# zhuhaozh/metadrive_ped

Hardware: AMD Instinct MI355X
Metric: agent-steps/sec at 4096 envs x 240-beam lidar (higher is better)
Workload: dtype f32; 1 GPU; BASELINE configs[1]: 4096 batched MetaDriveEnv per GPU, 3-block PG map (reference default block distribution: curves, straights, ramps, X/T intersections, roundabouts), 240-beam lidar, traffic_density=0.1, trigger traffic, auto-reset; envs_per_gpu=4096, agents_per_env=1, mover_capacity=24, n_beams=240

## Files before the change

### include/md_entity.h

```cpp
#ifndef MD_ENTITY_H
#define MD_ENTITY_H

#include <stddef.h>

#include "md_geom.h"
#include "md_lane_change.h"

MD_HD int md_scene_of_env(const MdState* g, int e) { return g->scene_of ? g->scene_of[e] : e; }
MD_HD size_t md_track_stride(const MdState* s, const MdConfig* c) {
    return (size_t)(s->walk.n_scenes > 0 ? s->walk.n_scenes : c->n_envs) * (size_t)c->cap;
}
MD_HD int md_scene(const MdState* s, int e) { return s->scene_of ? s->scene_of[0] : e; }

MD_HD MdState md_env_view(const MdState* g, const MdConfig* c, int e) {
    MdState v = *g;
    const size_t b = (size_t)e * (size_t)c->cap;
    const size_t bs = (size_t)md_scene_of_env(g, e) * (size_t)c->cap;
    const size_t a = (size_t)e * (size_t)c->agents_per_env;
    v.shape = g->shape + b;
    v.dyn = g->dyn ? g->dyn + b : 0;
    v.param = g->param ? g->param + b : 0;
    v.nav = g->nav ? g->nav + b : 0;
    v.pid = g->pid ? g->pid + b : 0;
    v.action = g->action ? g->action + 2 * b : 0;
// ... 118 lines not shown
    s->action[2 * n] = steer;
    s->action[2 * n + 1] = thr;
    float yaw = (sh->s * d->last_c - sh->c * d->last_s) / (float)c->substeps;
    d->last_x = sh->cx;
    d->last_y = sh->cy;
    d->last_c = sh->c;
    d->last_s = sh->s;
    d->steering = steer;
    d->throttle = thr;
    float x = sh->cx, y = sh->cy, psi = d->heading, v = d->speed;
    MdBicycle bike;
    md_bicycle_prepare(steer, thr, v, sh->hl, sh->hw, c->dt, c->enable_reverse && (sh->flags & MD_F_AGENT), &s->param[n], &bike);
    float c0, s0;
    md_sincos(psi, &s0, &c0);
    float cp = c0 * bike.cb - s0 * bike.sb, sp = s0 * bike.cb + c0 * bike.sb;
    for (int k = 0; k < c->substeps; ++k) md_bicycle_substep(&x, &y, &psi, &v, &cp, &sp, &yaw, thr, &bike, &s->param[n], c->dt);
    sh->cx = x;
    sh->cy = y;
    d->heading = psi;
    d->speed = v;
    md_sincos(psi, &sh->s, &sh->c);
}


#define MD_OBS_TASKS 9

typedef struct MdObsCtx {
    const MdLane *lane, *ref0, *ref_last, *next0, *fin, *rl;
    float cur_w, cur_n, positive_road;
    int valid;
    int cur_block;
} MdObsCtx;

MD_HD void md_observe_ctx(const MdLane* lanes, const MdRoad* roads, const MdState* s, int n, MdObsCtx* k) {
    const MdShape* sh = &s->shape[n];
    const MdNav* nav = &s->nav[n];
    k->valid = md_drives(sh->flags) && nav->lane >= 0;
    k->lane = k->ref0 = k->ref_last = k->next0 = k->fin = k->rl = lanes;
    k->cur_w = k->cur_n = k->positive_road = 0.0f;
    k->cur_block = 0;
    if (!k->valid) return;
    const MdRoad* cur_road = &roads[nav->road0];
    k->cur_block = cur_road->block_kind;
    int has_next = nav->ck1 != nav->ck0;
    const MdRoad* next_road = has_next ? &roads[nav->road1] : cur_road;
    k->lane = &lanes[nav->lane];
    k->ref0 = &lanes[cur_road->first_lane];
    k->ref_last = &lanes[cur_road->first_lane + cur_road->n_lanes - 1];
    k->next0 = &lanes[next_road->first_lane];
    k->fin = &lanes[s->final_lane[n]];
    k->cur_w = k->lane->width;
    k->cur_n = (float)cur_road->n_lanes;
    k->positive_road = 1.0f;
    if (k->lane->road == nav->road0) k->rl = k->lane;
    else {
        k->rl = k->ref0;
        k->positive_road = cur_road->negative ? -1.0f : 1.0f;
    }
}

MD_HD void md_observe_task(int task, const MdObsCtx* k, const MdState* s, const MdConfig* c, int n, float* out5) {
    const MdShape* sh = &s->shape[n];
    const MdDyn* d = &s->dyn[n];
    float x = sh->cx, y = sh->cy;
    out5[0] = out5[1] = out5[2] = out5[3] = out5[4] = 0.0f;
    if (!k->valid) return;
    if (task == 0 || task == 2 || task == 5 || task == 6 || task == 7) {
        const MdLane* L = (task == 0) ? k->ref0 : ((task == 2) ? k->lane : ((task == 5) ? k->fin : k->rl));
        float px = (task == 6) ? d->last_x : x;
        float py = (task == 6) ? d->last_y : y;
        md_lane_local(L, px, py, &out5[0], &out5[1]);
    } else if (task == 3 || task == 4) {
        md_navi_for_checkpoint((task == 3) ? k->ref0 : k->next0, (k->cur_n / 2.0f - 0.5f) * k->cur_w, x, y, sh->c, sh->s,
                               k->cur_n, k->cur_w, c->curve_radius_max, c->curve_angle_max, out5);
    } else if (task == 1) {
        out5[0] = md_heading_diff(k->ref_last, x, y, sh->c, sh->s);
    } else if (task == 8) {
        float cosb = (sh->c * d->last_c + sh->s * d->last_s) / (md_norm(sh->c, sh->s) * md_norm(d->last_c, d->last_s));
        float beta = md_acos(md_clip(cosb, 0.0f, 1.0f));
        out5[0] = md_clip(beta / 0.1f, 0.0f, 1.0f);
        out5[1] = md_step_energy(md_fabs(d->speed) * 3.6f, md_norm(d->last_x - x, d->last_y - y));
    }
}

#define MD_OBS_LANES 16
#if defined(__HIP_DEVICE_COMPILE__)
#define MD_LANE_IN(lane, mask) __extension__({ unsigned long long m_; __asm__ volatile("s_mov_b64 %0, %1" : "=s"(m_) : "i"(mask)); __builtin_amdgcn_inverse_ballot_w64(m_); })
#else
#define MD_LANE_IN(lane, mask) ((((mask) >> (lane)) & 1ull) != 0)
#endif
#define MD_LANE_F(m) ((int)(offsetof(MdLane, m) / sizeof(float)))

// ... 123 lines not shown
    if (MD_LANE_IN(lane, MD_LY)) {
        num3 = ac_hi ? 2.0f * md_asin_small(n3) : MD_HALF_PI_F - md_asin_small(cosb);
        den3 = 0.1f;
    }
    if (MD_LANE_IN(lane, MD_LE)) {
        float t = 3.25f * md_exp(0.01f * (md_fabs(speed) * 3.6f));
        num3 = t * q1;
        den3 = 100.0f;
    }
    const float q3 = num3 / den3;

    int w0 = task * 5;
    MD_PICK2(MD_LN, out0, (q3 + 1.0f) / 2.0f, w0, w0 + (lane >= 10));
    MD_PICK(MD_LH, out0, (!(ln * n2 != 0.0f)) ? 0.0f : md_clip(q3, -1.0f, 1.0f) / 2.0f + 0.5f);
    MD_PICK(MD_LY, out0, q3);
    MD_PICK2(MD_LE, out0, q3 * 1000.0f, w0, w0 + 1);
    MD_PICK(MD_LB, w0, w0 + 2);
    MD_PICK(MD_LA, w0, w0 + 4);

    MD_PICK(0xFD18ull, out0, md_clip(out0, 0.0f, 1.0f));
    if (MD_LANE_IN(lane, 0xFFFFull)) r45[w0] = out0;
    if (MD_LANE_IN(lane, MD_LF | MD_LB)) r45[w0 + 1] = (lane >= 12) ? md_clip(out1, 0.0f, 1.0f) : out1;
#undef MD_PICK
#undef MD_PICK2
#undef MD_LF
#undef MD_LN
#undef MD_LH
#undef MD_LY
#undef MD_LE
#undef MD_LB
#undef MD_LA
}

MD_HD void md_route_borders(const MdObsCtx* k, const float (*r)[5], float* to_left, float* to_right) {
    *to_left = r[0][1] + k->cur_w / 2.0f;
    *to_right = k->cur_w * k->cur_n - *to_left;
}

MD_HD void md_observe_state_dims(const MdObsCtx* k, const MdState* s, const MdConfig* c, int n, const float (*r)[5], float* obs) {
    const MdDyn* d = &s->dyn[n];
    const int o_mid = md_obs_mid(c), o_ll = md_obs_ll(c), o_navi = md_obs_navi(c);
    float to_left, to_right;
    md_route_borders(k, r, &to_left, &to_right);
    float speed_kmh = md_fabs(d->speed) * 3.6f;
    const MdParam* P = &s->param[n];
    const int o_base = md_obs_base(c);
    if (o_base) {
        obs[0] = md_clip(2.0f * s->shape[n].hl / 10.0f, 0.0f, 1.0f);
        obs[1] = md_clip(2.0f * s->shape[n].hw / 2.5f, 0.0f, 1.0f);
    }
    if (c->n_side <= 0) {
        obs[o_base + 0] = md_clip(to_left / c->total_width, 0.0f, 1.0f);
        obs[o_base + 1] = md_clip(to_right / c->total_width, 0.0f, 1.0f);
    }
    obs[o_mid + 0] = r[1][0];
    obs[o_mid + 1] = md_clip((speed_kmh + 1.0f) / (P->max_speed_kmh + 1.0f), 0.0f, 1.0f);
    obs[o_mid + 2] = md_clip((d->steering / 60.0f + 1.0f) / 2.0f, 0.0f, 1.0f);
    obs[o_mid + 3] = md_clip((s->action[2 * n] + 1.0f) / 2.0f, 0.0f, 1.0f);
    obs[o_mid + 4] = md_clip((s->action[2 * n + 1] + 1.0f) / 2.0f, 0.0f, 1.0f);
    obs[o_mid + 5] = r[8][0];
    float llat = r[2][1];
    if (c->n_lane_line <= 0) obs[o_ll] = md_clip((llat * 2.0f / c->max_lane_width + 1.0f) / 2.0f, 0.0f, 1.0f);
    if (!md_is_tollgate(c))
        for (int i = 0; i < 5; ++i) {
            obs[o_navi + i] = r[3][i];
            obs[o_navi + 5 + i] = r[4][i];
        }
}

MD_HD void md_observe_combine(const MdObsCtx* k, const MdState* s, const MdConfig* c, int a, int env_just_reset,
                              const float (*r)[5]) {
    int n = a;
    int just_reset = env_just_reset || ((s->shape[n].flags & MD_F_SPAWNED) != 0);
    s->shape[n].flags &= ~MD_F_SPAWNED;
    int ai = a;
    float* obs = s->obs + (size_t)ai * c->obs_dim;
    float* info = s->step_info + (size_t)ai * 8;
    MdDyn* d = &s->dyn[n];
    MdNav* nav = &s->nav[n];
    const int toll = md_is_tollgate(c);
    if (!k->valid) {
        if (s->done_out) ((uint32_t*)s->done_out)[ai] = 0u;
        for (int i = 0; i < md_obs_lidar(c); ++i) obs[i] = 0.0f;
        for (int i = c->obs_dim - md_obs_tail(c); i < c->obs_dim; ++i) obs[i] = 0.0f;
        s->reward[ai] = 0.0f;
        s->cost[ai] = 0.0f;
        for (int i = 0; i < 8; ++i) info[i] = 0.0f;
        return;
    }
    float cur_w = k->cur_w, cur_n = k->cur_n;

    float to_left, to_right;
    md_route_borders(k, r, &to_left, &to_right);
    uint32_t fl = s->flags[n] & (MD_FL_CRASH_VEHICLE | MD_FL_CRASH_OBJECT | MD_FL_CRASH_HUMAN | MD_FL_CRASH_BUILDING |
                                 MD_FL_CRASH_SIDEWALK | MD_FL_ON_WHITE_CONT | MD_FL_ON_YELLOW_CONT | MD_FL_ON_BROKEN |
                                 MD_FL_ON_CROSSWALK | MD_FL_ON_LANE);
    if (to_right < 0.0f || to_left < 0.0f) fl |= MD_FL_OUT_OF_ROUTE;

    md_observe_state_dims(k, s, c, n, r, obs);
    float speed_kmh = md_fabs(d->speed) * 3.6f;
    const MdParam* P = &s->param[n];
    float ls = r[2][0], llat = r[2][1];

    float fs = r[5][0], flat = r[5][1];
    int arrive = (k->fin->length - 5.0f < fs) && (fs < k->fin->length + 5.0f) && (cur_w / 2.0f >= flat) &&
                 (flat >= (0.5f - cur_n) * cur_w);
    int out_of_road = !(fl & MD_FL_ON_LANE);
    if (c->out_of_route_done) out_of_road = out_of_road || (fl & MD_FL_OUT_OF_ROUTE);
    else if (c->on_continuous_line_done)
        out_of_road = out_of_road || (fl & (MD_FL_ON_YELLOW_CONT | MD_FL_ON_WHITE_CONT | MD_FL_CRASH_SIDEWALK));
    if (toll) {
        out_of_road = (fl & MD_FL_CRASH_SIDEWALK) != 0;
        if (c->on_continuous_line_done) out_of_road = out_of_road || (fl & MD_FL_ON_YELLOW_CONT);
    }
    if (c->is_multi_agent && c->ma_kind == MD_MA_PARKING_LOT)
        out_of_road = !(fl & MD_FL_ON_LANE) || (fl & (MD_FL_ON_YELLOW_CONT | MD_FL_CRASH_SIDEWALK));
    const int racing = c->is_multi_agent && c->ma_kind == MD_MA_RACING;
    if (racing)
        out_of_road = ls < -5.0f;
    if (arrive) fl |= MD_FL_ARRIVE_DEST;
    if (out_of_road) fl |= MD_FL_OUT_OF_ROAD;

    float positive_road = k->positive_road;
    float long_last = r[6][0], long_now = r[7][0], lateral_now = r[7][1];
    float lateral_factor = 1.0f;
    if (c->use_lateral_reward) lateral_factor = md_clip(1.0f - 2.0f * md_fabs(lateral_now) / cur_w, 0.0f, 1.0f);
    float reward = 0.0f;
    if (toll) {
        reward += c->driving_reward * (long_now - long_last) * lateral_factor;
        if (k->cur_block == '$') {
            if (k->lane->speed_limit < speed_kmh) reward = -c->overspeed_penalty * speed_kmh / P->max_speed_kmh;
        } else reward += c->speed_reward * (speed_kmh / P->max_speed_kmh);
    } else {
        reward += c->driving_reward * (long_now - long_last) * lateral_factor * positive_road;
        reward += c->speed_reward * (speed_kmh / P->max_speed_kmh) * positive_road;
    }
    float step_reward = reward;
    int idle = 0;
    if (racing && !just_reset && s->idle_ring) {
        float* ring = s->idle_ring + (size_t)ai * MD_IDLE_WINDOW;
        int cnt = nav->toll_state;
        ring[cnt % MD_IDLE_WINDOW] = md_fabs(long_now - long_last);
        cnt += 1;
        if (cnt >= 2 * MD_IDLE_WINDOW) cnt -= MD_IDLE_WINDOW;
        nav->toll_state = cnt;
        if (cnt >= MD_IDLE_WINDOW) {
            float sum = 0.0f;
            for (int i = 0; i < MD_IDLE_WINDOW; ++i) sum += ring[(cnt + i) % MD_IDLE_WINDOW];
            idle = sum < 0.1f;
        }
    }
    if (arrive) reward = c->success_reward;
    else if (out_of_road) reward = -c->out_of_road_penalty;
    else if (fl & MD_FL_CRASH_VEHICLE) reward = -c->crash_vehicle_penalty;
    else if (racing) {
        if (fl & MD_FL_CRASH_SIDEWALK) reward = -c->crash_sidewalk_penalty;
        else if (idle) reward = -c->idle_penalty;
    } else if (fl & MD_FL_CRASH_OBJECT) reward = -c->crash_object_penalty;

    float cost = 0.0f;
    if (out_of_road) cost = c->out_of_road_cost;
    else if (fl & MD_FL_CRASH_VEHICLE) cost = c->crash_vehicle_cost;
    else if (fl & MD_FL_CRASH_OBJECT) cost = c->crash_object_cost;

// ... 37 lines not shown
        if (max_step) fl |= MD_FL_TRUNCATED;
    }
    s->flags[n] = fl;
    s->reward[ai] = reward;
    s->cost[ai] = cost;
    if (s->done_out) ((uint32_t*)s->done_out)[ai] = md_done_word(fl);
    if (toll) {
        int t = nav->toll_state & 0xffffff, last = (nav->toll_state >> 24) & 0xff;
        const int cur = k->cur_block, in_toll = (cur == '$');
        if (in_toll) t += 1;
        obs[c->obs_dim - 2] = in_toll ? 1.0f : 0.0f;
        obs[c->obs_dim - 1] = (in_toll && t > c->min_pass_steps) ? 1.0f : 0.0f;
        if (last && last != cur) {
            if (in_toll) nav->toll_entry = nav->steps + 1;
            else if ((cur == 'y' || cur == 'Y') && last == '$') nav->toll_exit = nav->steps + 1;
        }
        last = cur;
        nav->toll_state = t | (last << 24);
    }

    float step_energy = just_reset ? 0.0f : r[8][1];
    s->pid[n].energy += step_energy;
    info[0] = step_reward;
    info[1] = md_fabs(d->speed);
    info[2] = step_energy;
    info[3] = s->pid[n].energy;
    info[4] = just_reset ? 0.0f : info[4] + reward;
    info[5] = just_reset ? 0.0f : info[5] + cost;
    (void)llat;
    info[6] = ls;
    info[7] = (float)nav->steps;
    if (c->auto_reset && !c->is_multi_agent && !just_reset && (fl & (MD_FL_TERMINATED | MD_FL_TRUNCATED)))
        s->need_reset[0] = 1;
}

MD_HD void md_observe_agent(const MdLane* lanes, const MdRoad* roads, const MdState* s, const MdConfig* c, int a,
                             int just_reset) {
    MdObsCtx k;
    float r[MD_OBS_TASKS][5];
    md_observe_ctx(lanes, roads, s, a, &k);
    for (int t = 0; t < MD_OBS_TASKS; ++t) md_observe_task(t, &k, s, c, a, r[t]);
    md_observe_combine(&k, s, c, a, just_reset, (const float (*)[5])r);
}

typedef struct {
    int front[3], back[3];
    float front_d[3], back_d[3];
    int exist[3];
} FrontBack;

typedef struct {
    int success;
    int use_ref;
    int fail;
    int ids[3];
} MdIdmPlan;

#define IDM_MAX_LONG_DIST 30.0f
#define IDM_SAFE_LANE_CHANGE 15.0f
#define IDM_LANE_CHANGE_FREQ 50
#define IDM_LANE_CHANGE_SPEED_INC 10.0f
#define IDM_NORMAL_SPEED 30.0f
#define IDM_CREEP_SPEED 5.0f
#define IDM_MAX_SPEED 100.0f

MD_HD int md_road_connects(const MdWorld* w, int m, int from_node, int to_node) {
// ... 614 lines not shown
```

### metadrive_ped_amd/csrc/mdstep.hip

```cpp
#include <hip/hip_runtime.h>
#include <stddef.h>
#include <stdint.h>
#include <stdio.h>
#include <stdlib.h>

#include <type_traits>

#include "md_curriculum.h"
#include "md_expert.h"
#include "md_expert_sense.h"
#include "md_ai_protect.h"
#include "md_scenario.h"
#include "md_topdown.h"
#include "md_render.h"
#include "md_branch.h"
#include "md_ped.h"
#include "md_vector_obs.h"

namespace {

constexpr int kBlock = 256;

enum Phase : int {
    PH_RESET = 1,
// ... 8 lines not shown
    PH_ALL = 511,
    PH_LOCALIZE_ROAD_FIRST = PH_LOCALIZE | (1 << 20),
};

thread_local char g_err[256] = "ok";

#ifdef MD_STAMP
__device__ unsigned long long* g_stamp_buf = nullptr;
__device__ const int* g_env_order = nullptr;
#define MD_STAMP_AT(i)                                                                         \
    do {                                                                                       \
        if (threadIdx.x == 0 && g_stamp_buf) {                                                 \
            unsigned long long* sb_ = g_stamp_buf + (size_t)blockIdx.x * 32;                   \
            sb_[(i)] = __builtin_readcyclecounter();                                           \
            if ((i) == 0) {                                                                    \
                sb_[12] = __builtin_amdgcn_s_memrealtime();                                    \
                sb_[14] = (unsigned long long)__builtin_amdgcn_s_getreg(63492) |               \
                          ((unsigned long long)__builtin_amdgcn_s_getreg(63508) << 32);        \
            }                                                                                  \
            if ((i) == 11) sb_[13] = __builtin_amdgcn_s_memrealtime();                         \
        }                                                                                      \
    } while (0)
#define MD_FINE_STAMP(cond, i)                                                                 \
    do {                                                                                       \
        if ((cond) && g_stamp_buf) g_stamp_buf[(size_t)blockIdx.x * 32 + 16 + (i)] = __builtin_readcyclecounter(); \
    } while (0)
#define MD_LOC_COUNT(cond, hit)                                                                \
    do {                                                                                       \
        if ((cond) && g_stamp_buf) {                                                           \
            atomicAdd(&g_stamp_buf[(size_t)blockIdx.x * 32 + 16 + 12], 1ull);                  \
            if (hit) atomicAdd(&g_stamp_buf[(size_t)blockIdx.x * 32 + 16 + 13], 1ull);         \
        }                                                                                      \
    } while (0)
#else
#define MD_STAMP_AT(i) do { } while (0)
#define MD_FINE_STAMP(cond, i) do { } while (0)
#define MD_LOC_COUNT(cond, hit) do { } while (0)
#endif
#ifndef MD_ENV_SKIP
#define MD_ENV_SKIP 0
#endif

__host__ __device__ constexpr uint32_t align_up(uint32_t b, uint32_t a) { return (b + a - 1) & ~(a - 1); }

__device__ __forceinline__ float bcast_f(float v, int src) { return __shfl(v, src, 64); }
__device__ __forceinline__ int bcast_i(int v, int src) { return __shfl(v, src, 64); }

__device__ __forceinline__ void wave_lds_sync() {
    __builtin_amdgcn_fence(__ATOMIC_RELEASE, "wavefront");
    __builtin_amdgcn_wave_barrier();
    __builtin_amdgcn_fence(__ATOMIC_ACQUIRE, "wavefront");
}

#ifndef MD_NT_STAGE
#define MD_NT_STAGE 1
#endif
typedef unsigned int md_u32x4 __attribute__((ext_vector_type(4)));
__device__ __forceinline__ uint4 ld_stream(const uint4* p) {
#if MD_NT_STAGE
    const md_u32x4 v = __builtin_nontemporal_load(reinterpret_cast<const md_u32x4*>(p));
    return make_uint4(v.x, v.y, v.z, v.w);
#else
    return *p;
#endif
}
__device__ __forceinline__ void st_stream(uint4* p, const uint4 v) {
#if MD_NT_STAGE
    md_u32x4 t;
    t.x = v.x; t.y = v.y; t.z = v.z; t.w = v.w;
    __builtin_nontemporal_store(t, reinterpret_cast<md_u32x4*>(p));
// ... 1285 lines not shown
    const int my_slot = j0 + lane_id;
    const bool mine = (mask >> lane_id) & 1ull;
    MdIdmPlan plan;
    plan.success = plan.use_ref = plan.fail = 0;
    plan.ids[0] = plan.ids[1] = plan.ids[2] = -1;
    if (mine) md_idm_plan(&w, lanes, roads, &s, &c, m, my_slot, &plan);
    FrontBack fb;
    front_back_clear(fb);
    unsigned long long todo = mask;
    while (todo) {
        const int v = __ffsll((long long)todo) - 1;
        todo &= todo - 1;
        MdIdmPlan up;
        up.success = bcast_i(plan.success, v);
        up.use_ref = bcast_i(plan.use_ref, v);
        up.fail = bcast_i(plan.fail, v);
        up.ids[0] = bcast_i(plan.ids[0], v);
        up.ids[1] = bcast_i(plan.ids[1], v);
        up.ids[2] = bcast_i(plan.ids[2], v);
        FrontBack ufb;
        idm_scan_wave(lanes, s, c, j0 + v, lane_id, wave_list, up, ufb);
        wave_lds_sync();
        if (lane_id == v) {
            plan.fail = up.fail;
            fb = ufb;
        }
    }
    if (mine) md_idm_decide(lanes, roads, &s, my_slot, &plan, &fb);
}

#ifndef MD_OBS_LOCKSTEP
#define MD_OBS_LOCKSTEP 1
#endif
template <bool kLockstep = false>
__device__ __forceinline__ void observe_agent_wave1(const MdLane* lanes, const MdRoad* roads, const MdState& s, const MdConfig& c, int a,
                                    int just_reset, int lane_id, float* wave_scratch ) {
    MdObsCtx k;
    MD_FINE_STAMP(a == 0 && lane_id == 0, 8);
    md_observe_ctx(lanes, roads, &s, a, &k);
    MD_FINE_STAMP(a == 0 && lane_id == 0, 9);
    if constexpr (kLockstep) {
        if (lane_id < MD_OBS_TASKS * 5) wave_scratch[lane_id] = 0.0f;
        md_observe_lane(lane_id, &k, &s, &c, a, wave_scratch);
    } else if (lane_id < MD_OBS_TASKS) {
        float mine[5];
        md_observe_task(lane_id, &k, &s, &c, a, mine);
#pragma unroll
        for (int i = 0; i < 5; ++i) wave_scratch[lane_id * 5 + i] = mine[i];
    }
    wave_lds_sync();
    MD_FINE_STAMP(a == 0 && lane_id == 0, 10);
    if (lane_id == 0) md_observe_combine(&k, &s, &c, a, just_reset, (const float (*)[5])wave_scratch);
    __builtin_amdgcn_wave_barrier();
    MD_FINE_STAMP(a == 0 && lane_id == 0, 11);
}

constexpr int kObsGroups = 4;
constexpr int kObsScratch = kObsGroups * 48;

__device__ __forceinline__ void observe_agent_wave(const MdLane* lanes, const MdRoad* roads, const MdState& s, const MdConfig& c, int a_base,
                                   int just_reset, int lane_id, float* wave_scratch ) {
    const int g = lane_id >> 4, sub = lane_id & 15;
    const int a = a_base + g;
    const bool live = a < c.agents_per_env;
    float* scratch = wave_scratch + g * 48;
    MdObsCtx k;
    if (live) md_observe_ctx(lanes, roads, &s, a, &k);
    if (live && sub < MD_OBS_TASKS) {
        float mine[5];
        md_observe_task(sub, &k, &s, &c, a, mine);
#pragma unroll
// ... 302 lines not shown
__host__ __device__ inline EnvLds env_lds(int cap, int agents, int n_lanes, int n_roads, int waves, bool multi, bool lidar_only) {
    EnvLds L;
    L.shape = 0;
    L.dyn = L.shape + (uint32_t)cap * sizeof(MdShape);
    L.nav = L.dyn + (uint32_t)cap * sizeof(MdDyn);
    L.pid = L.nav + (uint32_t)cap * sizeof(MdNav);
    L.action = L.pid + (uint32_t)cap * sizeof(MdPid);
    L.flags = L.action + (uint32_t)cap * 2 * sizeof(float);
    L.lanes = align_up(L.flags + (uint32_t)cap * sizeof(uint32_t), 16);
    L.roads = L.lanes + (uint32_t)n_lanes * sizeof(MdLane);
    L.scratch = L.roads + (uint32_t)n_roads * sizeof(MdRoad);
    L.param = L.scratch + (uint32_t)waves * (multi ? kObsScratch : 48) * sizeof(float);
    L.final_lane = L.param + (uint32_t)cap * sizeof(MdParam);
    L.det = L.final_lane + align_up(cap, 2) * sizeof(int32_t);
    L.onlane = L.det + (uint32_t)agents * 2 * sizeof(unsigned long long);
    L.cfl = L.onlane + (uint32_t)cap * sizeof(uint32_t);
    const uint32_t shared_words = 2 * cap > 8 ? 2 * cap : 8;
    L.tk = L.onlane + shared_words * sizeof(uint32_t);
    L.bytes = lidar_only ? L.dyn : L.tk + 3 * sizeof(int);
    return L;
}

template <int PH, bool STAGE_MAP, bool RESPAWN = false, bool MULTI = false, int BLK = MD_ENV_BLOCK>
__global__ __launch_bounds__(BLK)
__attribute__((amdgpu_waves_per_eu(env_waves_per_eu<PH, RESPAWN, MULTI>() ? env_waves_per_eu<PH, RESPAWN, MULTI>() : 1,
                                   env_waves_per_eu<PH, RESPAWN, MULTI>() ? env_waves_per_eu<PH, RESPAWN, MULTI>() : 8)))
void env_kernel(MdWorld w, MdState g, MdConfig c, float* lidar_out,
                                                  int lidar_stride, int lidar_offset) {
    constexpr int kBlock = BLK;
    constexpr int kWaves = kBlock / 64;
    constexpr bool kIdmKeys = !STAGE_MAP && !RESPAWN && !MULTI;
    constexpr bool kLocRoadFirst = PH == PH_ALL ? kIdmKeys : PH == PH_LOCALIZE_ROAD_FIRST;
    constexpr bool kObsLockstep = MD_OBS_LOCKSTEP && PH == PH_ALL && kIdmKeys;
    if constexpr (PH == PH_ALL && !RESPAWN && !MULTI && !STAGE_MAP) lean_pins_fold(g, c);
    if ((int)blockIdx.x >= c.n_envs) return;
#ifdef MD_STAMP
    const int e = g_env_order ? g_env_order[blockIdx.x] : (int)blockIdx.x;
#else
    const int e = blockIdx.x;
#endif
    const int tid = threadIdx.x;
    const int wave = tid >> 6, lane = tid & 63;
    const int cap = c.cap;

    const int n_stage_lanes = STAGE_MAP ? w.max_lanes : 0, n_stage_roads = STAGE_MAP ? w.max_roads : 0;
    constexpr bool kLidarOnly = (PH == PH_LIDAR);
    const EnvLds L = env_lds(cap, c.agents_per_env, n_stage_lanes, n_stage_roads, kWaves, MULTI, kLidarOnly);
    extern __shared__ __attribute__((aligned(16))) unsigned char smem[];
    MdShape* l_shape = reinterpret_cast<MdShape*>(smem + L.shape);
    MdDyn* l_dyn = reinterpret_cast<MdDyn*>(smem + L.dyn);
    MdNav* l_nav = reinterpret_cast<MdNav*>(smem + L.nav);
    MdPid* l_pid = reinterpret_cast<MdPid*>(smem + L.pid);
    float* l_action = reinterpret_cast<float*>(smem + L.action);
    uint32_t* l_flags = reinterpret_cast<uint32_t*>(smem + L.flags);
    MdLane* l_lanes = reinterpret_cast<MdLane*>(smem + L.lanes);
    MdRoad* l_roads = reinterpret_cast<MdRoad*>(smem + L.roads);
    float* l_scratch = reinterpret_cast<float*>(smem + L.scratch) + wave * (MULTI ? kObsScratch : 48);
    MdParam* l_param = reinterpret_cast<MdParam*>(smem + L.param);
    int32_t* l_final = reinterpret_cast<int32_t*>(smem + L.final_lane);
    unsigned long long* l_det = reinterpret_cast<unsigned long long*>(smem + L.det);
    const EnvImage img = {l_shape, l_dyn, l_pid, l_param, l_nav, l_action, l_flags, l_final};
    uint32_t* l_onlane = reinterpret_cast<uint32_t*>(smem + L.onlane);
    uint32_t* l_cfl = reinterpret_cast<uint32_t*>(smem + L.cfl);
    int* l_tk = reinterpret_cast<int*>(smem + L.tk);
    const bool track_det = (PH == PH_ALL) && (RESPAWN || MULTI) && g.detected != nullptr;

// ... 89 lines not shown
        copy16(l_dyn, gv.dyn0, cap * (int)sizeof(MdDyn), tid, kBlock);
        copy16(l_nav, gv.nav0, cap * (int)sizeof(MdNav), tid, kBlock);
        copy16(l_pid, gv.pid0, cap * (int)sizeof(MdPid), tid, kBlock);
        if (MULTI && c.random_agent_model && gv.param0)
            copy16(l_param, gv.param0, cap * (int)sizeof(MdParam), tid, kBlock);
        for (int j = tid; j < cap; j += kBlock) {
            l_action[2 * j] = 0.0f;
            l_action[2 * j + 1] = 0.0f;
            l_flags[j] = 0u;
        }
        if (MULTI || (RESPAWN && (c.traffic_mode == 1 || c.traffic_mode == 2))) {
            for (int i = tid; i < cap * MD_ROUTE_LEN; i += kBlock) {
                gv.route_nodes[i] = gv.route_nodes0[i];
                gv.route_roads[i] = gv.route_roads0[i];
            }
            for (int j = tid; j < cap; j += kBlock) l_final[j] = gv.final_lane0[j];
        }
        if (MULTI) {
            for (int j = tid; j < cap; j += kBlock) gv.agent_id[j] = j;
            if (tid == 0) {
                gv.env_steps[0] = 0;
                int n0 = 0;
                for (int j = 0; j < c.agents_per_env; ++j) n0 += (gv.shape0[j].flags & MD_F_ALIVE) ? 1 : 0;
                gv.next_agent_id[0] = n0;
            }
        }
    }
    MdState s = local_view(gv, img);
    if (kLidarOnly) {
        s = gv;
        s.shape = l_shape;
    }
    if ((MULTI || PH == PH_ALL) && tid == 0) l_tk[0] = l_tk[1] = l_tk[2] = 0;
    __syncthreads();
    MD_STAMP_AT(1);
    constexpr bool kTriggerEarly = MD_TRIGGER_EARLY && PH == PH_ALL && kIdmKeys && kWaves > 1;
    constexpr int kTrigWord = (kWaves - 1) * 48 + 46;
    if (kTriggerEarly && wave == kWaves - 1) {
        int min_order, trig_road;
        trigger_search_wave(s, c, lane, &min_order, &trig_road);
        if (lane == 0) {
            int* l_trig = reinterpret_cast<int*>(smem + L.scratch) + kTrigWord;
            l_trig[0] = min_order;
            l_trig[1] = trig_road;
        }
    }

    if ((PH & PH_LIFECYCLE) && MULTI && !just_reset) {
        lifecycle_block(w, s, c, w.env_map[e], tid, kBlock, reinterpret_cast<int*>(l_onlane));
    }

    constexpr bool kFused = (PH == PH_ALL);
    const bool agent_idm = (kFused && !RESPAWN && !MULTI) ? false : (c.agent_idm == MD_AGENT_IDM);
    const bool lane_change = (RESPAWN || MULTI) && c.agent_idm == MD_AGENT_LANE_CHANGE;
    constexpr bool kPlanAhead = kFused && kWaves > 1 && !MULTI;
    const bool plan_ahead = kPlanAhead && !agent_idm;
    if ((PH & PH_IDM) && !just_reset && !plan_ahead) {
        if (wave == 0) trigger_env(lanes, s, c, lane);
        __syncthreads();
        MD_STAMP_AT(2);
        for (int j = (agent_idm ? 0 : c.agents_per_env) + wave; j < cap; j += kWaves) {
            const int f = s.shape[j].flags;
            if (md_drives(f) && (agent_idm || !(f & MD_F_AGENT))) idm_vehicle_wave<kIdmKeys>(w, lanes, roads, s, c, w.env_map[e], j, lane, reinterpret_cast<int*>(l_scratch));
        }
        __syncthreads();
    }
// ... 6 lines not shown
            }
            if (RESPAWN) md_advance_mover(&s, &c, j);
            else md_integrate_mover(&s, &c, j);
        }
        if (!RESPAWN)
            for (int j = tid; j < cap; j += kBlock) md_walk_mover(&s, &c, j);
        __syncthreads();
    }
    MD_STAMP_AT(4);
    unsigned long long drv_lo = 0ull, drv_hi = 0ull;
    if (kFused) {
        const SlotMask drv = drive_mask(s.shape, cap, lane);
        drv_lo = drv.lo;
        drv_hi = drv.hi;
        const SlotMask adrv = agent_share(drv, c.agents_per_env);
        const unsigned long long adrv_lo = adrv.lo, adrv_hi = adrv.hi;
        const int nd = popc(drv), na = popc(adrv);
        if (MULTI) {
            const int npair = (nd + 1) >> 1;
            for (int guard = 0; guard < npair + na; ++guard) {
                int item = 0;
                if (lane == 0) item = atomicAdd(&l_tk[0], 1);
                item = __builtin_amdgcn_readfirstlane(item);
                if (item < 0 || item >= npair + na) break;
                if (item < na) contacts_vehicle(w, s, c, e, kth_bit(adrv_lo, adrv_hi, item), lane, l_cfl);
                else localize_pair(w, lanes, roads, s, e, kth_bit(drv_lo, drv_hi, 2 * (item - na)), kth_bit(drv_lo, drv_hi, 2 * (item - na) + 1), lane, l_onlane);
            }
        } else if (nd + na <= kWaves) {
            for (int item = wave; item < nd + na; item += kWaves) {
                if (item < nd) {
                    if (!(MD_ENV_SKIP & 4)) localize_vehicle<kLocRoadFirst>(w, lanes, roads, s, e, kth_bit(drv_lo, drv_hi, item), lane, l_onlane);
                } else if (!(MD_ENV_SKIP & 8)) contacts_vehicle(w, s, c, e, kth_bit(adrv_lo, adrv_hi, item - nd), lane, l_cfl);
            }
        } else {
            const int npair = (nd + 1) >> 1;
            for (int item = wave; item < npair + na; item += kWaves) {
                if (item < npair) {
                    if (!(MD_ENV_SKIP & 4)) localize_pair<kLocRoadFirst>(w, lanes, roads, s, e, kth_bit(drv_lo, drv_hi, 2 * item), kth_bit(drv_lo, drv_hi, 2 * item + 1), lane, l_onlane);
                } else if (!(MD_ENV_SKIP & 8))
                    contacts_vehicle(w, s, c, e, kth_bit(adrv_lo, adrv_hi, item - npair), lane, l_cfl);
            }
        }
        __syncthreads();
    } else {
        if (PH & PH_LOCALIZE) {
            for (int j = wave; j < cap; j += kWaves) localize_vehicle<kLocRoadFirst>(w, lanes, roads, s, e, j, lane);
            __syncthreads();
        }
        MD_STAMP_AT(5);
        if (PH & PH_CONTACTS) {
            for (int j = wave; j < cap; j += kWaves) contacts_vehicle(w, s, c, e, j, lane);
            __syncthreads();
        }
    }
    MD_STAMP_AT(6);
    if (PH & PH_TRAFFIC) {
        for (int j = tid; j < cap; j += kBlock) {
            const bool drove = kFused ? ((((j < 64) ? (drv_lo >> j) : (drv_hi >> (j - 64))) & 1ull) != 0ull) : false;
            if (kFused && !drove) continue;
            const int f = s.shape[j].flags;
            if (kFused)
                s.flags[j] = l_onlane[j] | ((f & MD_F_AGENT) ? l_cfl[j] : 0u);
            if (md_drives(f) && !(f & MD_F_AGENT) && !(s.flags[j] & MD_FL_ON_LANE)) {
                s.shape[j].flags = f & ~MD_F_ALIVE;
                if (kFused) l_cfl[j] = kRemovedMark;
            }
        }
        if (plan_ahead && wave == kWaves - 1) {
            if (kTriggerEarly) {
                const int* l_trig = reinterpret_cast<const int*>(smem + L.scratch) + kTrigWord;
                trigger_fire_wave(lanes, s, c, lane, __builtin_amdgcn_readfirstlane(l_trig[0]), __builtin_amdgcn_readfirstlane(l_trig[1]));
            } else trigger_env(lanes, s, c, lane);
        }
        __syncthreads();
        if (RESPAWN) {
            if (tid == 0) md_traffic_respawn_env(&w, lanes, &s, &c, w.env_map[e]);
            __syncthreads();
        }
    }
    MD_STAMP_AT(7);
    if (plan_ahead) {
        if (wave == 0) {
            if (!(MD_ENV_SKIP & 16))
                for (int a = 0; a < c.agents_per_env; ++a) observe_agent_wave1<kObsLockstep>(lanes, roads, s, c, a, just_reset, lane, l_scratch);
        } else if (!(MD_ENV_SKIP & 2)) {
            int rank = 0;
            for (int j0 = 0; j0 < cap; j0 += 64) {
                const int jl = j0 + lane;
                const int fl = (jl < cap) ? s.shape[jl].flags : 0;
                unsigned long long mk = __ballot(jl < cap && md_drives(fl) && !(fl & MD_F_AGENT));
                while (mk) {
                    const int j = j0 + __ffsll((long long)mk) - 1;
                    mk &= mk - 1;
                    if (rank % (kWaves - 1) == wave - 1) idm_vehicle_wave<kIdmKeys>(w, lanes, roads, s, c, w.env_map[e], j, lane, reinterpret_cast<int*>(l_scratch));
                    ++rank;
                }
            }
        }
        MD_STAMP_AT(8);
    } else if (PH & PH_OBSERVE) {
        if (MULTI) {
            const int n_grp = (c.agents_per_env + kObsGroups - 1) / kObsGroups;
            for (int guard = 0; guard < n_grp; ++guard) {
                int gi = 0;
                if (lane == 0) gi = atomicAdd(&l_tk[1], 1);
                gi = __builtin_amdgcn_readfirstlane(gi);
                if (gi < 0 || gi >= n_grp) break;
                observe_agent_wave(lanes, roads, s, c, gi * kObsGroups, just_reset, lane, l_scratch);
            }
        } else {
            for (int a = wave; a < c.agents_per_env; a += kWaves) observe_agent_wave1(lanes, roads, s, c, a, just_reset, lane, l_scratch);
        }
        MD_STAMP_AT(8);
    }
    if ((PH & PH_LIDAR) && !(PH == PH_ALL && (MD_ENV_SKIP & 1))) {
        if (c.n_beams > 0) phase_lidar(w, s, c, e, tid, kWaves, lidar_out, lidar_stride, lidar_offset, track_det ? l_det : nullptr, PH == PH_ALL ? &l_tk[2] : nullptr);
    }
// ... 1606 lines not shown
```

Measured before the change: 59.42 million agent-steps/s.

## Speculatively compute agent observation lanes on an idle wave during localize phase

When the localize/contacts phase leaves a wave idle, that wave precomputes the ego agent's per-lane observation tasks using the nav key as it stands at that moment, and caches the context in shared scratch. Later, the observe step checks whether the nav key is unchanged. On a hit it skips recomputing the context and lanes and only runs the combine step. This moves observation work off the critical path, at the cost of extra shared-memory words, a key comparison, and wasted work on a miss. It adds a possible ordering hazard, because localize may update nav concurrently, so it relies on the key check and volatile reads to stay correct.

Measured after the change: 60.56 million agent-steps/s (median of 6 runs). 1.9% higher.

```diff
diff --git a/include/md_entity.h b/include/md_entity.h
--- a/include/md_entity.h
+++ b/include/md_entity.h
@@ -174,32 +174,58 @@
     int cur_block;
 } MdObsCtx;
 
+typedef struct MdObsKey {
+    int32_t lane, road0, road1, ck0, ck1;
+} MdObsKey;
+#define MD_OBS_KEY_WORDS 5
+
+MD_HD void md_obs_key_of(const MdNav* nav, MdObsKey* q) {
+    q->lane = nav->lane;
+    q->road0 = nav->road0;
+    q->road1 = nav->road1;
+    q->ck0 = nav->ck0;
+    q->ck1 = nav->ck1;
+}
+
+MD_HD int md_obs_key_same(const MdObsKey* q, const MdNav* nav) {
+    return q->lane == nav->lane && q->road0 == nav->road0 && q->road1 == nav->road1 && q->ck0 == nav->ck0 && q->ck1 == nav->ck1;
+}
+
+#define MD_OBSERVE_CTX_BODY(NAV)                                                                    \
+    const MdShape* sh = &s->shape[n];                                                               \
+    k->valid = md_drives(sh->flags) && (NAV)->lane >= 0;                                            \
+    k->lane = k->ref0 = k->ref_last = k->next0 = k->fin = k->rl = lanes;                            \
+    k->cur_w = k->cur_n = k->positive_road = 0.0f;                                                  \
+    k->cur_block = 0;                                                                               \
+    if (!k->valid) return;                                                                          \
+    const MdRoad* cur_road = &roads[(NAV)->road0];                                                  \
+    k->cur_block = cur_road->block_kind;                                                            \
+    int has_next = (NAV)->ck1 != (NAV)->ck0;                                                        \
+    const MdRoad* next_road = has_next ? &roads[(NAV)->road1] : cur_road;                           \
+    k->lane = &lanes[(NAV)->lane];                                                                  \
+    k->ref0 = &lanes[cur_road->first_lane];                                                         \
+    k->ref_last = &lanes[cur_road->first_lane + cur_road->n_lanes - 1];                             \
+    k->next0 = &lanes[next_road->first_lane];                                                       \
+    k->fin = &lanes[s->final_lane[n]];                                                              \
+    k->cur_w = k->lane->width;                     \
+    k->cur_n = (float)cur_road->n_lanes;                                                            \
+                                                        \
+    k->positive_road = 1.0f;                                                                        \
+    if (k->lane->road == (NAV)->road0) k->rl = k->lane;                                             \
+    else {                                                                                          \
+        k->rl = k->ref0;                                                                            \
+        k->positive_road = cur_road->negative ? -1.0f : 1.0f;                                       \
+    }
+
+MD_HD void md_observe_ctx_of(const MdLane* lanes, const MdRoad* roads, const MdState* s, int n, const MdObsKey* q, MdObsCtx* k) {
+    MD_OBSERVE_CTX_BODY(q)
+}
+
 MD_HD void md_observe_ctx(const MdLane* lanes, const MdRoad* roads, const MdState* s, int n, MdObsCtx* k) {
-    const MdShape* sh = &s->shape[n];
     const MdNav* nav = &s->nav[n];
-    k->valid = md_drives(sh->flags) && nav->lane >= 0;
-    k->lane = k->ref0 = k->ref_last = k->next0 = k->fin = k->rl = lanes;
-    k->cur_w = k->cur_n = k->positive_road = 0.0f;
-    k->cur_block = 0;
-    if (!k->valid) return;
-    const MdRoad* cur_road = &roads[nav->road0];
-    k->cur_block = cur_road->block_kind;
-    int has_next = nav->ck1 != nav->ck0;
-    const MdRoad* next_road = has_next ? &roads[nav->road1] : cur_road;
-    k->lane = &lanes[nav->lane];
-    k->ref0 = &lanes[cur_road->first_lane];
-    k->ref_last = &lanes[cur_road->first_lane + cur_road->n_lanes - 1];
-    k->next0 = &lanes[next_road->first_lane];
-    k->fin = &lanes[s->final_lane[n]];
-    k->cur_w = k->lane->width;
-    k->cur_n = (float)cur_road->n_lanes;
-    k->positive_road = 1.0f;
-    if (k->lane->road == nav->road0) k->rl = k->lane;
-    else {
-        k->rl = k->ref0;
-        k->positive_road = cur_road->negative ? -1.0f : 1.0f;
-    }
-}
+    MD_OBSERVE_CTX_BODY(nav)
+}
+#undef MD_OBSERVE_CTX_BODY
 
 MD_HD void md_observe_task(int task, const MdObsCtx* k, const MdState* s, const MdConfig* c, int n, float* out5) {
     const MdShape* sh = &s->shape[n];
@@ -389,16 +415,20 @@
 #undef MD_LA
 }
 
+MD_HD void md_route_borders_of(float cur_w, float cur_n, const float (*r)[5], float* to_left, float* to_right) {
+    *to_left = r[0][1] + cur_w / 2.0f;
+    *to_right = cur_w * cur_n - *to_left;
+}
+
 MD_HD void md_route_borders(const MdObsCtx* k, const float (*r)[5], float* to_left, float* to_right) {
-    *to_left = r[0][1] + k->cur_w / 2.0f;
-    *to_right = k->cur_w * k->cur_n - *to_left;
-}
-
-MD_HD void md_observe_state_dims(const MdObsCtx* k, const MdState* s, const MdConfig* c, int n, const float (*r)[5], float* obs) {
+    md_route_borders_of(k->cur_w, k->cur_n, r, to_left, to_right);
+}
+
+MD_HD void md_observe_state_dims_of(float cur_w, float cur_n, const MdState* s, const MdConfig* c, int n, const float (*r)[5], float* obs) {
     const MdDyn* d = &s->dyn[n];
     const int o_mid = md_obs_mid(c), o_ll = md_obs_ll(c), o_navi = md_obs_navi(c);
     float to_left, to_right;
-    md_route_borders(k, r, &to_left, &to_right);
+    md_route_borders_of(cur_w, cur_n, r, &to_left, &to_right);
     float speed_kmh = md_fabs(d->speed) * 3.6f;
     const MdParam* P = &s->param[n];
     const int o_base = md_obs_base(c);
@@ -425,8 +455,20 @@
         }
 }
 
-MD_HD void md_observe_combine(const MdObsCtx* k, const MdState* s, const MdConfig* c, int a, int env_just_reset,
-                              const float (*r)[5]) {
+MD_HD void md_observe_state_dims(const MdObsCtx* k, const MdState* s, const MdConfig* c, int n, const float (*r)[5], float* obs) {
+    md_observe_state_dims_of(k->cur_w, k->cur_n, s, c, n, r, obs);
+}
+
+typedef struct MdObsHand {
+    int valid;
+    float cur_w, cur_n, positive_road;
+    int cur_block;
+    const float* fin_length;
+    const float* lane_speed_limit;
+} MdObsHand;
+
+MD_HD void md_observe_combine_of(const MdObsHand* k, const MdState* s, const MdConfig* c, int a, int env_just_reset,
+                                 const float (*r)[5]) {
     int n = a;
     int just_reset = env_just_reset || ((s->shape[n].flags & MD_F_SPAWNED) != 0);
     s->shape[n].flags &= ~MD_F_SPAWNED;
@@ -448,19 +490,19 @@
     float cur_w = k->cur_w, cur_n = k->cur_n;
 
     float to_left, to_right;
-    md_route_borders(k, r, &to_left, &to_right);
+    md_route_borders_of(k->cur_w, k->cur_n, r, &to_left, &to_right);
     uint32_t fl = s->flags[n] & (MD_FL_CRASH_VEHICLE | MD_FL_CRASH_OBJECT | MD_FL_CRASH_HUMAN | MD_FL_CRASH_BUILDING |
                                  MD_FL_CRASH_SIDEWALK | MD_FL_ON_WHITE_CONT | MD_FL_ON_YELLOW_CONT | MD_FL_ON_BROKEN |
                                  MD_FL_ON_CROSSWALK | MD_FL_ON_LANE);
     if (to_right < 0.0f || to_left < 0.0f) fl |= MD_FL_OUT_OF_ROUTE;
 
-    md_observe_state_dims(k, s, c, n, r, obs);
+    md_observe_state_dims_of(k->cur_w, k->cur_n, s, c, n, r, obs);
     float speed_kmh = md_fabs(d->speed) * 3.6f;
     const MdParam* P = &s->param[n];
     float ls = r[2][0], llat = r[2][1];
 
     float fs = r[5][0], flat = r[5][1];
-    int arrive = (k->fin->length - 5.0f < fs) && (fs < k->fin->length + 5.0f) && (cur_w / 2.0f >= flat) &&
+    int arrive = (*k->fin_length - 5.0f < fs) && (fs < *k->fin_length + 5.0f) && (cur_w / 2.0f >= flat) &&
                  (flat >= (0.5f - cur_n) * cur_w);
     int out_of_road = !(fl & MD_FL_ON_LANE);
     if (c->out_of_route_done) out_of_road = out_of_road || (fl & MD_FL_OUT_OF_ROUTE);
@@ -486,7 +528,7 @@
     if (toll) {
         reward += c->driving_reward * (long_now - long_last) * lateral_factor;
         if (k->cur_block == '$') {
-            if (k->lane->speed_limit < speed_kmh) reward = -c->overspeed_penalty * speed_kmh / P->max_speed_kmh;
+            if (*k->lane_speed_limit < speed_kmh) reward = -c->overspeed_penalty * speed_kmh / P->max_speed_kmh;
         } else reward += c->speed_reward * (speed_kmh / P->max_speed_kmh);
     } else {
         reward += c->driving_reward * (long_now - long_last) * lateral_factor * positive_road;
@@ -590,6 +632,12 @@
     info[7] = (float)nav->steps;
     if (c->auto_reset && !c->is_multi_agent && !just_reset && (fl & (MD_FL_TERMINATED | MD_FL_TRUNCATED)))
         s->need_reset[0] = 1;
+}
+
+MD_HD void md_observe_combine(const MdObsCtx* k, const MdState* s, const MdConfig* c, int a, int env_just_reset,
+                              const float (*r)[5]) {
+    const MdObsHand h = {k->valid, k->cur_w, k->cur_n, k->positive_road, k->cur_block, &k->fin->length, &k->lane->speed_limit};
+    md_observe_combine_of(&h, s, c, a, env_just_reset, r);
 }
 
 MD_HD void md_observe_agent(const MdLane* lanes, const MdRoad* roads, const MdState* s, const MdConfig* c, int a,
diff --git a/metadrive_ped_amd/csrc/mdstep.hip b/metadrive_ped_amd/csrc/mdstep.hip
--- a/metadrive_ped_amd/csrc/mdstep.hip
+++ b/metadrive_ped_amd/csrc/mdstep.hip
@@ -64,10 +64,21 @@
             if (hit) atomicAdd(&g_stamp_buf[(size_t)blockIdx.x * 32 + 16 + 13], 1ull);         \
         }                                                                                      \
     } while (0)
+#define MD_AHEAD_STAMP(cond, i)                                                                \
+    do {                                                                                       \
+        if ((cond) && g_stamp_buf) g_stamp_buf[(size_t)blockIdx.x * 32 + (i)] = __builtin_readcyclecounter(); \
+    } while (0)
+enum : int { MD_AHEAD_EVALUATED = 32, MD_AHEAD_HIT = 40, MD_AHEAD_MISS = 48 };
+#define MD_AHEAD_COUNT(cond, what)                                                             \
+    do {                                                                                       \
+        if ((cond) && g_stamp_buf) atomicAdd(&g_stamp_buf[(size_t)blockIdx.x * 32 + 16 + 12], 1ull << (what)); \
+    } while (0)
 #else
 #define MD_STAMP_AT(i) do { } while (0)
 #define MD_FINE_STAMP(cond, i) do { } while (0)
 #define MD_LOC_COUNT(cond, hit) do { } while (0)
+#define MD_AHEAD_STAMP(cond, i) do { } while (0)
+#define MD_AHEAD_COUNT(cond, what) do { } while (0)
 #endif
 #ifndef MD_ENV_SKIP
 #define MD_ENV_SKIP 0
@@ -1419,11 +1430,73 @@
 #ifndef MD_OBS_LOCKSTEP
 #define MD_OBS_LOCKSTEP 1
 #endif
-template <bool kLockstep = false>
+enum ObsAheadWord : int {
+    kAhMark = 45,
+    kAhLane = 46, kAhRoad0 = 47, kAhRoad1 = 2, kAhCk0 = 3, kAhCk1 = 4,
+    kAhValid = 6, kAhCurW = 7, kAhCurN = 8, kAhPosRoad = 9, kAhFinLen = 12
+};
+#ifndef MD_OBS_AHEAD
+#define MD_OBS_AHEAD 1
+#endif
+__device__ __forceinline__ void observe_ahead_wave(const MdLane* lanes, const MdRoad* roads, const MdState& s, const MdConfig& c, int lane_id,
+                                                   float* scratch0 ) {
+    constexpr int a = 0;
+    MD_AHEAD_STAMP(lane_id == 0, 2);
+    const volatile int32_t* nv = reinterpret_cast<const volatile int32_t*>(&s.nav[a]);
+    MdObsKey q;
+    q.lane = __builtin_amdgcn_readfirstlane(nv[offsetof(MdNav, lane) / 4]);
+    q.road0 = __builtin_amdgcn_readfirstlane(nv[offsetof(MdNav, road0) / 4]);
+    q.road1 = __builtin_amdgcn_readfirstlane(nv[offsetof(MdNav, road1) / 4]);
+    q.ck0 = __builtin_amdgcn_readfirstlane(nv[offsetof(MdNav, ck0) / 4]);
+    q.ck1 = __builtin_amdgcn_readfirstlane(nv[offsetof(MdNav, ck1) / 4]);
+    MdObsCtx k;
+    md_observe_ctx_of(lanes, roads, &s, a, &q, &k);
+    if (lane_id < MD_OBS_TASKS * 5) scratch0[lane_id] = 0.0f;
+    md_observe_lane(lane_id, &k, &s, &c, a, scratch0);
+    if (lane_id == 0) {
+        int* w = reinterpret_cast<int*>(scratch0);
+        w[kAhLane] = q.lane;
+        w[kAhRoad0] = q.road0;
+        w[kAhRoad1] = q.road1;
+        w[kAhCk0] = q.ck0;
+        w[kAhCk1] = q.ck1;
+        w[kAhValid] = k.valid;
+        scratch0[kAhCurW] = k.cur_w;
+        scratch0[kAhCurN] = k.cur_n;
+        scratch0[kAhPosRoad] = k.positive_road;
+        scratch0[kAhFinLen] = k.fin->length;
+        w[kAhMark] = 1;
+    }
+    MD_AHEAD_COUNT(lane_id == 0, MD_AHEAD_EVALUATED);
+    MD_AHEAD_STAMP(lane_id == 0, 5);
+}
+
+template <bool kLockstep = false, bool kAhead = false>
 __device__ __forceinline__ void observe_agent_wave1(const MdLane* lanes, const MdRoad* roads, const MdState& s, const MdConfig& c, int a,
                                     int just_reset, int lane_id, float* wave_scratch ) {
     MdObsCtx k;
     MD_FINE_STAMP(a == 0 && lane_id == 0, 8);
+    if constexpr (kAhead) {
+        if (a == 0) {
+            const int* w = reinterpret_cast<const int*>(wave_scratch);
+            const MdObsKey q = {w[kAhLane], w[kAhRoad0], w[kAhRoad1], w[kAhCk0], w[kAhCk1]};
+            const int hit = w[kAhMark] != 0 && md_obs_key_same(&q, &s.nav[a]);
+            if (__builtin_amdgcn_readfirstlane(hit)) {
+                MD_AHEAD_COUNT(lane_id == 0, MD_AHEAD_HIT);
+                MD_FINE_STAMP(lane_id == 0, 9);
+                MD_FINE_STAMP(lane_id == 0, 10);
+                if (lane_id == 0) {
+                    const MdObsHand h = {w[kAhValid], wave_scratch[kAhCurW], wave_scratch[kAhCurN], wave_scratch[kAhPosRoad], 0,
+                                         &wave_scratch[kAhFinLen], nullptr};
+                    md_observe_combine_of(&h, &s, &c, a, just_reset, (const float (*)[5])wave_scratch);
+                }
+                __builtin_amdgcn_wave_barrier();
+                MD_FINE_STAMP(lane_id == 0, 11);
+                return;
+            }
+            MD_AHEAD_COUNT(lane_id == 0, MD_AHEAD_MISS);
+        }
+    }
     md_observe_ctx(lanes, roads, &s, a, &k);
     MD_FINE_STAMP(a == 0 && lane_id == 0, 9);
     if constexpr (kLockstep) {
@@ -1792,6 +1865,7 @@
     constexpr bool kIdmKeys = !STAGE_MAP && !RESPAWN && !MULTI;
     constexpr bool kLocRoadFirst = PH == PH_ALL ? kIdmKeys : PH == PH_LOCALIZE_ROAD_FIRST;
     constexpr bool kObsLockstep = MD_OBS_LOCKSTEP && PH == PH_ALL && kIdmKeys;
+    constexpr bool kObsAhead = MD_OBS_AHEAD && kObsLockstep && kWaves > 1;
     if constexpr (PH == PH_ALL && !RESPAWN && !MULTI && !STAGE_MAP) lean_pins_fold(g, c);
     if ((int)blockIdx.x >= c.n_envs) return;
 #ifdef MD_STAMP
@@ -1947,6 +2021,7 @@
         s.shape = l_shape;
     }
     if ((MULTI || PH == PH_ALL) && tid == 0) l_tk[0] = l_tk[1] = l_tk[2] = 0;
+    if (kObsAhead && tid == 0) reinterpret_cast<int*>(smem + L.scratch)[kAhMark] = 0;
     __syncthreads();
     MD_STAMP_AT(1);
     constexpr bool kTriggerEarly = MD_TRIGGER_EARLY && PH == PH_ALL && kIdmKeys && kWaves > 1;
@@ -2019,6 +2094,10 @@
                     if (!(MD_ENV_SKIP & 4)) localize_vehicle<kLocRoadFirst>(w, lanes, roads, s, e, kth_bit(drv_lo, drv_hi, item), lane, l_onlane);
                 } else if (!(MD_ENV_SKIP & 8)) contacts_vehicle(w, s, c, e, kth_bit(adrv_lo, adrv_hi, item - nd), lane, l_cfl);
             }
+            if constexpr (kObsAhead) {
+                if (nd + na < kWaves && wave == nd + na && !(MD_ENV_SKIP & 16))
+                    observe_ahead_wave(lanes, roads, s, c, lane, reinterpret_cast<float*>(smem + L.scratch));
+            }
         } else {
             const int npair = (nd + 1) >> 1;
             for (int item = wave; item < npair + na; item += kWaves) {
@@ -2069,7 +2148,7 @@
     if (plan_ahead) {
         if (wave == 0) {
             if (!(MD_ENV_SKIP & 16))
-                for (int a = 0; a < c.agents_per_env; ++a) observe_agent_wave1<kObsLockstep>(lanes, roads, s, c, a, just_reset, lane, l_scratch);
+                for (int a = 0; a < c.agents_per_env; ++a) observe_agent_wave1<kObsLockstep, kObsAhead>(lanes, roads, s, c, a, just_reset, lane, l_scratch);
         } else if (!(MD_ENV_SKIP & 2)) {
             int rank = 0;
             for (int j0 = 0; j0 < cap; j0 += 64) {
```
